# 0xMiden/miden-vm

Hardware: AMD Instinct MI355X
Metric: trace rows/sec proved (2^20-row trace, 96-bit sec) (higher is better)
Workload: dtype u64 (Goldilocks field, p = 2^64 - 2^32 + 1); 1 GPU; full proof of miden:20:51:8 (DummyMidenAir 2^20 x 51 + 8 EF aux), 96-bit production PCS params (blowup 8, FRI arity 4, 27 queries, PoW 4/12/16), Poseidon2 LMCS; trace resident in HBM, transcript on host; log_trace_rows=20, main_width=51, aux_width_ef=8, log_blowup=3, proof_bytes=137697, parallelism=1 GPU

## Files before the change

miden-vm_amd/csrc/ntt.hip:

```cpp
#include "ctx.hpp"
#include "gl.cuh"
#include "kernels.hpp"
#include "poseidon2_fast.cuh"
#include <utility>

#ifndef NTT_ASM_MUL
#define NTT_ASM_MUL 2
#endif
#if P2F_ASM && NTT_ASM_MUL == 1
#define NTT_MUL1 p2f_mul
#elif P2F_ASM && NTT_ASM_MUL == 2
#define NTT_MUL1 p2f_mul_nv
#else
#define NTT_MUL1 p2f_mul_c
#endif

static constexpr int NTT_TILE_LOG = 12;
static constexpr int NTT_TILE_LOG_BIG = 14;
static constexpr int NTT_THREADS = 256;
static int ntt_tile_log(int log_n) {
  static const int big_max = [] {
    const char* e = getenv("MH_NTT_BIG_MAX");
    return e ? atoi(e) : 22;
  }();
  return log_n > 20 && log_n <= big_max ? NTT_TILE_LOG_BIG : NTT_TILE_LOG;
}

static bool ntt_coef_rot(int log_n) {
  static const int on = [] { const char* e = getenv("MH_NTT_ROT"); return e ? atoi(e) : 1; }();
  return on && log_n >= NTT_TILE_LOG && ntt_tile_log(log_n) == NTT_TILE_LOG;
}

struct PowTable {
  u64 pw[32];
};
__global__ void k_fill_powers(u64* out, size_t n, PowTable t, u64 scale) {
  size_t k = blockIdx.x * (size_t)blockDim.x + threadIdx.x;
  if (k >= n) return;
  u64 r = scale;
  size_t e = k;
#pragma unroll 1
  for (int i = 0; e; i++, e >>= 1)
    if (e & 1) r = gl_mul(r, t.pw[i]);
  out[k] = r;
}

static void fill_powers(mh_ctx* c, u64* out, size_t n, u64 base, u64 scale) {
  PowTable t;
  u64 b = base;
  for (int i = 0; i < 32; i++) {
    t.pw[i] = b;
    b = gl_sqr(b);
  }
  if (n == 0) return;
  MH_LAUNCH(k_fill_powers, dim3((n + 255) / 256), dim3(256), 0, c->stream, out, n, t, scale);
}

const u64* mh_ctx::twiddles(int log_n, bool inverse) {
  auto& m = inverse ? tw_inv : tw_fwd;
  auto it = m.find(log_n);
  if (it != m.end()) return it->second.u();
  size_t half = log_n ? ((size_t)1 << (log_n - 1)) : 1;
  DevBuf b(half * 8);
  u64 w = gl_two_adic_generator(log_n);
  if (inverse) w = gl_inv(w);
  fill_powers(this, b.u(), half, w, 1);
  const u64* p = b.u();
  m[log_n] = std::move(b);
  return p;
}

__global__ __launch_bounds__(256) void k_transpose_rm_to_cm(const u64* __restrict__ in, u64* __restrict__ out, size_t n,
                                                           size_t w) {
  __shared__ u64 tile[32][33];
  size_t r0 = (size_t)blockIdx.x * 32, c0 = (size_t)blockIdx.y * 32;
  int tx = threadIdx.x & 31, ty = threadIdx.x >> 5;
  for (int k = ty; k < 32; k += 8) {
    size_t r = r0 + k, cc = c0 + tx;
    if (r < n && cc < w) tile[k][tx] = in[r * w + cc];
  }
  __syncthreads();
  for (int k = ty; k < 32; k += 8) {
    size_t cc = c0 + k, r = r0 + tx;
    if (r < n && cc < w) out[cc * n + r] = gl_canon(tile[tx][k]);
  }
}

void launch_transpose_rm_to_cm(mh_ctx* c, const u64* in, u64* out, size_t n, size_t w, hipStream_t stream) {
  dim3 grid((unsigned)((n + 31) / 32), (unsigned)((w + 31) / 32));
  MH_LAUNCH(k_transpose_rm_to_cm, grid, dim3(256), 0, stream ? stream : c->stream, in, out, n, w);
}

struct NttPassArgs {
  const u64* src;
// ... 344 lines not shown
    t[i] = NttW{v0[f], v1[f], v2[f]};
    if (!INV) {
      if (S) t[i] = ntt_w_shl(pre ? ntt_w_from(ntt_w_fold1(ntt_w_bias(t[i]))) : t[i], S);
      p[i] = a[i];
      q[i] = t[i];
    } else {
      p[i] = E >= 96 ? t[i] : a[i];
      q[i] = E >= 96 ? a[i] : t[i];
    }
  }
  ntt_w_bflyN<N>(s, d, a, t, p, q);
#pragma unroll
  for (int i = 0; i < N; i++) {
    const int e = ntt_bfly_lo(M, K0 + i), f = e | (1 << M), j = e & ((1 << M) - 1);
    const int E = (W16 * (8 >> M) * j) % 192, S = E % 96;
    const bool pre = (FOLD >> (8 * M + j)) & 1u;
    NttW lo = s[i], hi = d[i];
    if (!INV) {
      if (E >= 96) { lo = d[i]; hi = s[i]; }
    } else if (S) {
      hi = ntt_w_shl(pre ? ntt_w_from(ntt_w_fold1(ntt_w_bias(hi))) : hi, S);
    }
    v0[e] = lo.w0; v1[e] = lo.w1; v2[e] = lo.w2;
    v0[f] = hi.w0; v1[f] = hi.w1; v2[f] = hi.w2;
  }
}
template <int G, bool INV, int I = 0>
__device__ __forceinline__ void ntt_w_stages(u32 (&v0)[1 << G], u32 (&v1)[1 << G], u32 (&v2)[1 << G]) {
  if constexpr (I < G) {
    constexpr int M = INV ? G - 1 - I : I, H = 1 << (G - 1), N = H < NTT_ILV ? H : NTT_ILV;
    ntt_w_stage_part<G, INV, M, 0, N>(v0, v1, v2);
    if constexpr (H > N) ntt_w_stage_part<G, INV, M, N, H - N>(v0, v1, v2);
    ntt_w_stages<G, INV, I + 1>(v0, v1, v2);
  }
}
template <int G, bool INV>
__device__ __forceinline__ void ntt_dft_wide(u64 (&x)[1 << G]) {
  u32 v0[1 << G], v1[1 << G], v2[1 << G];
#pragma unroll
  for (int e = 0; e < (1 << G); e++) { v0[e] = lo32(x[e]); v1[e] = hi32(x[e]); v2[e] = 0u; }
  const NttW z = ntt_w_bias(NttW{v0[0], v1[0], 0u});
  v0[0] = z.w0; v1[0] = z.w1; v2[0] = z.w2;
  ntt_w_stages<G, INV>(v0, v1, v2);
  constexpr int NF = (1 << G) < NTT_ILV ? (1 << G) : NTT_ILV;
#pragma unroll
  for (int c = 0; c < (1 << G); c += NF) {
    u64 r[NF];
    u32 f0[NF], f1[NF], f2[NF];
#pragma unroll
    for (int i = 0; i < NF; i++) { f0[i] = v0[c + i]; f1[i] = v1[c + i]; f2[i] = v2[c + i]; }
    ntt_w_foldN<NF>(r, f0, f1, f2);
#pragma unroll
    for (int i = 0; i < NF; i++) x[c + i] = r[i];
  }
}
#endif

template <int G, bool INV>
__device__ __forceinline__ void ntt_dft_regs(u64 (&x)[1 << G], bool dif) {
#if P2F_ASM && NTT_ASM_BFLY == 2
  ntt_dft_wide<G, INV>(x);
  return;
#elif P2F_ASM && NTT_ASM_BFLY
  if constexpr (!INV && G >= 3) {
    ntt_fwd_dft_asm<G>(x);
    return;
  }
#endif
  constexpr int W16 = INV ? 36 : 156;
  if (!dif) {
#pragma unroll
    for (int m = 0; m < G; m++)
#pragma unroll
      for (int e = 0; e < (1 << G); e++)
        if (!(e & (1 << m))) ntt_bfly_dit(x[e], x[e | (1 << m)], (W16 * (8 >> m) * (e & ((1 << m) - 1))) % 192);
  } else {
#pragma unroll
    for (int m = G - 1; m >= 0; m--)
#pragma unroll
      for (int e = 0; e < (1 << G); e++)
        if (!(e & (1 << m))) ntt_bfly_dif(x[e], x[e | (1 << m)], (W16 * (8 >> m) * (e & ((1 << m) - 1))) % 192);
  }
}
template <int K, int OFF>
__device__ __forceinline__ void ntt_tw_mul(u64* x, const u64* __restrict__ tw, int s, u32 gm) {
  if constexpr (K > 0) {
    constexpr int C = K >= 5 ? 5 : K;
    u64 a[C], b[C];
#pragma unroll
    for (int i = 0; i < C; i++) {
      a[i] = x[OFF + i];
      b[i] = (tw + ((size_t)(OFF + i - 1) << s))[gm];
    }
#if P2F_ASM && NTT_ASM_MUL == 1
    p2f_mulN<C>(a, a, b);
#else
#pragma unroll
    for (int i = 0; i < C; i++) a[i] = NTT_MUL1(a[i], b[i]);
#endif
#pragma unroll
    for (int i = 0; i < C; i++) x[OFF + i] = a[i];
    ntt_tw_mul<K - C, OFF + C>(x, tw, s, gm);
  }
}
#else
template <int K, int OFF>
__device__ void ntt_tw_mul(u64* x, const u64* __restrict__ tw, int s, u32 gm);
template <int G, bool INV>
__device__ void ntt_dft_regs(u64 (&x)[1 << G], bool dif);
__device__ u64 ntt_canon(u64 t);
__device__ u64 p2f_mul_c(u64 a, u64 b);
#endif

#ifndef NTT16_OCC
#define NTT16_OCC
#endif
#ifndef NTT_SWZ
#define NTT_SWZ 1
#endif
static size_t ntt_lds_bytes(int tile_log) {
  if (NTT_SWZ && tile_log == NTT_TILE_LOG) return ((size_t)1 << tile_log) * 8;
  return (((size_t)1 << tile_log) + ((size_t)1 << (tile_log - 4))) * 8;
}
template <bool SWZ>
__device__ __forceinline__ u32 ntt_pad(u32 l) {
  return SWZ ? (l ^ ((l >> 4) & 31u)) : (l + (l >> 4));
}

#define NTT_STORE(p, v) (*(p) = (v))
template <int G, bool INV, bool SWZ, int B0>
__device__ __forceinline__ void ntt_round(const NttPassArgs& a, u64* lds, int st, u32 tile_n, size_t lo0, u64* dst_direct,
                                          size_t gbase, const u64* __restrict__ tw, const u64* __restrict__ src_direct = nullptr,
                                          const u64* xin = nullptr) {
  const int b0 = B0 >= 0 ? B0 : st + a.cb, s = a.s_lo + st;
  const u32 cb_mask = (1u << a.cb) - 1;
  constexpr bool FAST = SWZ && B0 >= 0;
  for (u32 q = threadIdx.x; q < (tile_n >> G); q += blockDim.x) {
    const u32 low = q & ((1u << b0) - 1);
    const u32 l0 = ((q >> b0) << (b0 + G)) | low;
    const u32 gm = (((l0 >> a.cb) & ((1u << st) - 1)) << a.s_lo) | ((u32)lo0 << a.cb) | (l0 & cb_mask);
    const u32 p0 = ntt_pad<SWZ>(l0);
    char* const ldsb = reinterpret_cast<char*>(lds);
    const u32 pb = p0 * 8u, pb1 = (p0 ^ 16u) * 8u;
    auto slot = [&](int e) -> u64* {
      if constexpr (FAST && B0 == 8) return reinterpret_cast<u64*>(ldsb + ((e & 1) ? pb1 : pb) + ((u32)e << 11));
      else if constexpr (FAST) return reinterpret_cast<u64*>(ldsb + (pb ^ (ntt_pad<true>((u32)e << B0) * 8u)));
      else return lds + (SWZ ? (p0 ^ ntt_pad<true>((u32)e << b0)) : ntt_pad<false>(l0 | ((u32)e << b0)));
    };
    u64 x[1 << G];
    if (xin) {
#pragma unroll
      for (int e = 0; e < (1 << G); e++) x[e] = xin[e];
    } else if (src_direct) {
      const u32 six = (u32)(gbase | ((size_t)(l0 >> a.cb) << a.s_lo) | (l0 & cb_mask));
#pragma unroll
      for (int e = 0; e < (1 << G); e++) x[e] = (src_direct + ((size_t)e << s))[six];
    } else {
#pragma unroll
    for (int e = 0; e < (1 << G); e++) x[e] = *slot(e);
    }
    if (!INV && s > 0) ntt_tw_mul<(1 << G) - 1, 1>(x, tw, s, gm);
    ntt_dft_regs<G, INV>(x, INV);
    if (INV && s > 0) ntt_tw_mul<(1 << G) - 1, 1>(x, tw, s, gm);
    if (INV && dst_direct && a.rot && b0 == 0 && G == 4) {
      const u32 rix = (u32)gbase + (l0 >> 4);
#pragma unroll
      for (int e = 0; e < (1 << G); e++) NTT_STORE((dst_direct + ((size_t)e << 8)) + rix, a.canon_out ? ntt_canon(x[e]) : x[e]);
    } else if (dst_direct) {
      const u32 tix = (u32)(gbase | ((size_t)(l0 >> a.cb) << a.s_lo) | (l0 & cb_mask));
      if (a.canon_out) {
#pragma unroll
        for (int e = 0; e < (1 << G); e++) NTT_STORE((dst_direct + ((size_t)e << s)) + tix, ntt_canon(x[e]));
      } else {
#pragma unroll
        for (int e = 0; e < (1 << G); e++) NTT_STORE((dst_direct + ((size_t)e << s)) + tix, x[e]);
      }
    } else {
#pragma unroll
      for (int e = 0; e < (1 << G); e++) *slot(e) = x[e];
    }
  }
}

template <bool INV, int THREADS, int MODE = 0>
__global__ __launch_bounds__(THREADS) NTT16_OCC void k_ntt16_pass(NttPassArgs a) {
  extern __shared__ u64 lds[];
  constexpr bool SWZ = NTT_SWZ && THREADS == NTT_THREADS;
  const int tile_log = a.r_bits + a.cb;
  const u32 tile_n = 1u << tile_log;
  const u32 cb_mask = (1u << a.cb) - 1;
  const u32 tile = a.col_fastest ? blockIdx.y : blockIdx.x;
  const u32 col_id = a.col_fastest ? blockIdx.x : blockIdx.y;
  const int lo_bits = a.s_lo - a.cb;
  const size_t lo0 = tile & ((1u << lo_bits) - 1);
  const size_t hi = tile >> lo_bits;
  const size_t gbase = (hi << (a.s_lo + a.r_bits)) | (lo0 << a.cb);
  const u64* src0 = a.src + (size_t)col_id * a.src_col_stride;
  u64 raw[MODE == 1 ? 16 : 1];
  for (u32 z = 0; z < a.n_z; z++) {
  const u32 zc = blockIdx.z * a.n_z + z;
  const u32 srow = a.group_cols ? (col_id / a.group_cols) * a.group_z + zc : zc;
  u64* dst = a.dst + (size_t)col_id * a.dst_col_stride + (size_t)zc * a.dst_z_stride;
  const u64* src = src0 + (size_t)zc * a.src_z_stride;
  if (z) __syncthreads();

  constexpr int LOG_T = THREADS == 256 ? 8 : 10;
  const bool direct_first = MODE == 0 && THREADS == NTT_THREADS && a.direct_first && tile_n == 16u * THREADS;
  if (direct_first) {
  } else if (tile_n == 16u * THREADS && a.cb <= LOG_T) {
    const u32 tid = threadIdx.x;
    const u32 g0 = (u32)(gbase | ((size_t)(tid >> a.cb) << a.s_lo) | (tid & cb_mask));
    const int shg = LOG_T - a.cb + a.s_lo;
    const u32 p0 = ntt_pad<SWZ>(tid);
    if constexpr (MODE == 1) {
      if (z == 0) {
#pragma unroll
        for (int j = 0; j < 16; j++) raw[j] = (src + ((size_t)j << shg))[g0];
        if (a.scale_full) {
          const u64* sf = a.scale_full + ((size_t)srow << a.log_n);
#pragma unroll
          for (int c = 0; c < 16; c += 4) {
            u64 t[4];
#pragma unroll
            for (int j = 0; j < 4; j++) t[j] = (sf + ((size_t)(c + j) << shg))[g0];
#pragma unroll
            for (int j = 0; j < 4; j++) raw[c + j] = NTT_MUL1(raw[c + j], t[j]);
          }
        } else {
#pragma unroll 4
          for (int j = 0; j < 16; j++) {
            const u32 k = bitrev32(a.rot ? (g0 - tid) + ((tid << 4) | (u32)j) : g0 + ((u32)j << shg), a.log_n);
            const u64 sc = NTT_MUL1(a.scale_lo[srow * a.scale_lo_z + (k & ((1u << a.lb) - 1))], a.scale_hi[srow * a.scale_hi_z + (k >> a.lb)]);
            raw[j] = NTT_MUL1(raw[j], sc);
          }
        }
      } else {
#pragma unroll
        for (int c = 0; c < 16; c += 8) {
          u64 t[8];
#pragma unroll
          for (int j = 0; j < 8; j++) t[j] = (a.step + ((size_t)(c + j) << shg))[g0];
#pragma unroll
          for (int j = 0; j < 8; j++) raw[c + j] = NTT_MUL1(raw[c + j], t[j]);
        }
      }
      if (!a.rot) {
#pragma unroll
        for (int j = 0; j < 16; j++) lds[p0 ^ ntt_pad<true>((u32)j * THREADS)] = raw[j];
      }
    } else
    if (THREADS == NTT_THREADS && !a.scale_lo && !a.scale_full) {
      u64 v[16];
#pragma unroll
      for (int j = 0; j < 16; j++) v[j] = (src + ((size_t)j << shg))[g0];
#pragma unroll
      for (int j = 0; j < 16; j++)
        lds[SWZ ? (p0 ^ ntt_pad<true>((u32)j * THREADS)) : ntt_pad<false>(tid + (u32)j * THREADS)] = v[j];
    } else
#pragma unroll 1
    for (int c = 0; c < 16; c += 4) {
      u64 v[4];
#pragma unroll
      for (int j = 0; j < 4; j++) v[j] = (src + ((size_t)(c + j) << shg))[g0];
      if (a.scale_full) {
        const u64* sf = a.scale_full + ((size_t)srow << a.log_n);
#pragma unroll
        for (int j = 0; j < 4; j++) v[j] = NTT_MUL1(v[j], (sf + ((size_t)(c + j) << shg))[g0]);
      } else if (a.scale_lo) {
#pragma unroll
        for (int j = 0; j < 4; j++) {
          const u32 k = bitrev32(a.rot ? (g0 - tid) + ((tid << 4) | (u32)(c + j)) : g0 + ((u32)(c + j) << shg), a.log_n);
          const u64 sc = NTT_MUL1(a.scale_lo[srow * a.scale_lo_z + (k & ((1u << a.lb) - 1))], a.scale_hi[srow * a.scale_hi_z + (k >> a.lb)]);
          v[j] = NTT_MUL1(v[j], sc);
        }
      }
      if (a.rot) {
#pragma unroll
        for (int j = 0; j < 4; j++) lds[ntt_pad<SWZ>((tid << 4) | (u32)(c + j))] = v[j];
      } else
#pragma unroll
      for (int j = 0; j < 4; j++)
        lds[SWZ ? (p0 ^ ntt_pad<true>((u32)(c + j) * THREADS)) : ntt_pad<false>(tid + (u32)(c + j) * THREADS)] = v[j];
    }
  } else {
    for (u32 l = threadIdx.x; l < tile_n; l += THREADS) {
      size_t g = gbase | ((size_t)(l >> a.cb) << a.s_lo) | (l & cb_mask);
      u64 v = src[g];
      if (a.scale_full) {
        v = NTT_MUL1(v, a.scale_full[((size_t)srow << a.log_n) + g]);
      } else if (a.scale_lo) {
        u32 k = bitrev32((u32)g, a.log_n);
        u64 sc = NTT_MUL1(a.scale_lo[srow * a.scale_lo_z + (k & ((1u << a.lb) - 1))], a.scale_hi[srow * a.scale_hi_z + (k >> a.lb)]);
        v = NTT_MUL1(v, sc);
      }
      lds[ntt_pad<SWZ>(l)] = v;
    }
  }
  const bool regs_first = MODE == 1 && a.rot;
  if (!direct_first && !regs_first) __syncthreads();
  const int rem = a.r_bits & 3, n16 = a.r_bits >> 2;
  const int n_rounds = n16 + (rem ? 1 : 0);
  if (n_rounds == 0) {
    if (threadIdx.x == 0) dst[gbase] = ntt_canon(lds[0]);
    continue;
  }
  for (int i = 0; i < n_rounds; i++) {
    const int ri = INV ? n_rounds - 1 - i : i;
    int st, g;
    if (rem) {
      st = ri == 0 ? 0 : rem + 4 * (ri - 1);
      g = ri == 0 ? rem : 4;
    } else {
      st = 4 * ri;
      g = 4;
    }
    u64* direct = (i == n_rounds - 1) ? dst : nullptr;
    const int b0 = st + a.cb;
#define NTT_ROUND(GG, BB) ntt_round<GG, INV, SWZ, BB>(a, lds, st, tile_n, lo0, direct, gbase, a.tw_round[ri])
    if (direct_first && i == 0) ntt_round<4, INV, SWZ, INV ? 8 : 4>(a, lds, st, tile_n, lo0, direct, gbase, a.tw_round[ri], src);
    else if (regs_first && i == 0) ntt_round<4, INV, SWZ, 0>(a, lds, st, tile_n, lo0, direct, gbase, a.tw_round[ri], nullptr, raw);
    else if (g == 4 && b0 == 0) NTT_ROUND(4, 0);
    else if (g == 4 && b0 == 4) NTT_ROUND(4, 4);
    else if (g == 4 && b0 == 8) NTT_ROUND(4, 8);
    else if (g == 4) NTT_ROUND(4, -1);
    else if (g == 3) NTT_ROUND(3, -1);
    else if (g == 2) NTT_ROUND(2, -1);
    else NTT_ROUND(1, -1);
#undef NTT_ROUND
    if (!direct) __syncthreads();
  }
  }
}

struct PassPlan {
  int s_lo, r_bits, cb;
};
static std::vector<PassPlan> plan_passes(int log_n) {
  std::vector<PassPlan> p;
  const int T = ntt_tile_log(log_n);
  int c = log_n < T ? log_n : T;
  p.push_back({0, c, 0});
  int rem = log_n - c;
  if (rem > 0) {
    const int max_r = T - 4;
    int np = (rem + max_r - 1) / max_r;
    int s = c;
    for (int i = 0; i < np; i++) {
      int r = rem / np + (i < rem % np ? 1 : 0);
      p.push_back({s, r, T - r});
      s += r;
    }
  }
  return p;
}

static std::vector<std::pair<int, int>> pass_rounds(int r_bits) {
  std::vector<std::pair<int, int>> r;
  const int rem = r_bits & 3;
  int st = 0;
  if (rem) {
    r.push_back({0, rem});
    st = rem;
  }
  for (; st < r_bits; st += 4) r.push_back({st, 4});
  return r;
}
__global__ void k_fill_round_plane(u64* out, int s, int G, int log_n, PowTable t) {
  const size_t idx = blockIdx.x * (size_t)blockDim.x + threadIdx.x;
  if (idx >= ((size_t)((1 << G) - 1) << s)) return;
  const u32 e = (u32)(idx >> s) + 1;
  const size_t gm = idx & (((size_t)1 << s) - 1);
  const u32 rho = bitrev32(e, G);
  size_t ex = (gm * rho) << (log_n - s - G);
  u64 r = 1;
#pragma unroll 1
  for (int i = 0; ex; i++, ex >>= 1)
    if (ex & 1) r = gl_mul(r, t.pw[i]);
  out[idx] = r;
}
struct NttPlanes {
  const u64* base;
  std::vector<size_t> off;
};
static NttPlanes ntt_planes(mh_ctx* c, int log_n, bool inverse, const std::vector<PassPlan>& plan) {
  const std::string key = "nttp:" + std::to_string(log_n) + (inverse ? ":i" : ":f");
  auto it = c->tables.find(key);
  if (it == c->tables.end()) {
    std::vector<size_t> off(plan.size() * 4, 0);
    size_t total = 1;
    for (size_t i = 0; i < plan.size(); i++) {
      auto rounds = pass_rounds(plan[i].r_bits);
      for (size_t k = 0; k < rounds.size(); k++) {
        const int s = plan[i].s_lo + rounds[k].first, G = rounds[k].second;
        off[i * 4 + k] = total;
        if (s > 0) total += (size_t)((1 << G) - 1) << s;
      }
    }
    DevBuf b(total * 8);
    PowTable t;
    u64 w = gl_two_adic_generator(log_n);
    if (inverse) w = gl_inv(w);
    for (int i = 0; i < 32; i++) {
      t.pw[i] = w;
      w = gl_sqr(w);
    }
    for (size_t i = 0; i < plan.size(); i++) {
      auto rounds = pass_rounds(plan[i].r_bits);
      for (size_t k = 0; k < rounds.size(); k++) {
        const int s = plan[i].s_lo + rounds[k].first, G = rounds[k].second;
        if (s == 0) continue;
        const size_t cnt = (size_t)((1 << G) - 1) << s;
        MH_LAUNCH(k_fill_round_plane, dim3((unsigned)((cnt + 255) / 256)), dim3(256), 0, c->stream, b.u() + off[i * 4 + k], s, G,
                           log_n, t);
      }
    }
    c->table_index[key] = off;
    it = c->tables.emplace(key, std::move(b)).first;
  }
  return NttPlanes{it->second.u(), c->table_index[key]};
}

static void launch_pass(mh_ctx* c, NttPassArgs a, size_t n_cols, size_t n_z, bool one_coset_per_workgroup = false) {
  size_t tiles = (size_t)1 << (a.log_n - a.r_bits - a.cb);
  MH_REQUIRE(n_z >= 1 && (n_z & (n_z - 1)) == 0, "internal: the number of output cosets of a pass must be a power of two");
  size_t zsplit = 1;
  while (zsplit < n_z && (one_coset_per_workgroup || tiles * n_cols * zsplit < 4096)) zsplit *= 2;
  a.n_z = (u32)(n_z / zsplit);
  static const int colfast = [] { const char* e = getenv("MH_NTT_COLFAST"); return e ? atoi(e) : 1; }();
  a.col_fastest = (colfast && tiles <= 65535) ? 1 : 0;
  dim3 grid(a.col_fastest ? (unsigned)n_cols : (unsigned)tiles, a.col_fastest ? (unsigned)tiles : (unsigned)n_cols, (unsigned)zsplit);
  const int T = ntt_tile_log(a.log_n);
  const size_t lds = ntt_lds_bytes(T);
  if (T == NTT_TILE_LOG) {
    if (a.dif) MH_LAUNCH((k_ntt16_pass<true, NTT_THREADS>), grid, dim3(NTT_THREADS), lds, c->stream, a);
    else if (a.step && a.n_z > 1 && NTT_SWZ && a.r_bits + a.cb == NTT_TILE_LOG && a.cb == 0)
      MH_LAUNCH((k_ntt16_pass<false, NTT_THREADS, 1>), grid, dim3(NTT_THREADS), lds, c->stream, a);
    else MH_LAUNCH((k_ntt16_pass<false, NTT_THREADS>), grid, dim3(NTT_THREADS), lds, c->stream, a);
  } else {
    if (!c->ntt_big_lds_attr) {
      HIP_CHECK(hipFuncSetAttribute((const void*)k_ntt16_pass<true, 1024>, hipFuncAttributeMaxDynamicSharedMemorySize, (int)lds));
      HIP_CHECK(hipFuncSetAttribute((const void*)k_ntt16_pass<false, 1024>, hipFuncAttributeMaxDynamicSharedMemorySize, (int)lds));
      c->ntt_big_lds_attr = true;
    }
    if (a.dif) MH_LAUNCH((k_ntt16_pass<true, 1024>), grid, dim3(1024), lds, c->stream, a);
    else MH_LAUNCH((k_ntt16_pass<false, 1024>), grid, dim3(1024), lds, c->stream, a);
  }
}

void ntt_inverse_dif_inplace(mh_ctx* c, u64* cols, size_t n_cols, int log_n) { ntt_inverse_dif(c, cols, cols, n_cols, log_n); }

void ntt_inverse_dif(mh_ctx* c, const u64* src, u64* dst, size_t n_cols, int log_n) {
  if (log_n == 0) {
    if (src != dst) HIP_CHECK(hipMemcpyAsync(dst, src, n_cols * 8, hipMemcpyDeviceToDevice, c->stream));
    return;
  }
  auto plan = plan_passes(log_n);
  const NttPlanes tw = ntt_planes(c, log_n, true, plan);
  for (int i = (int)plan.size() - 1; i >= 0; i--) {
    NttPassArgs a{};
    a.src = (i == (int)plan.size() - 1) ? src : dst; a.dst = dst;
    a.src_col_stride = a.dst_col_stride = (size_t)1 << log_n;
    a.dst_z_stride = 0;
    a.log_n = log_n; a.s_lo = plan[i].s_lo; a.r_bits = plan[i].r_bits; a.cb = plan[i].cb;
    a.dif = 1; a.scale_lo = nullptr; a.scale_hi = nullptr;
    for (int k = 0; k < 4; k++) a.tw_round[k] = tw.base + tw.off[i * 4 + k];
    a.canon_out = 0;
    static const int direct = [] { const char* e = getenv("MH_NTT_DIRECT"); return e ? atoi(e) : 1; }();
    a.direct_first = direct && NTT_SWZ && a.r_bits >= 4 && a.r_bits + a.cb == NTT_TILE_LOG;
    a.rot = i == 0 && ntt_coef_rot(log_n);
    launch_pass(c, a, n_cols, 1);
  }
}

struct CosetTables {
  const u64* lo;
  const u64* hi;
  int lb;
};
static CosetTables coset_tables(mh_ctx* c, int log_n, const std::vector<u64>& bases, u64 post_scale) {
  CosetTables t;
  t.lb = (log_n + 1) / 2;
  const size_t nlo = (size_t)1 << t.lb, nhi = (size_t)1 << (log_n - t.lb);
  u64 h = 0xcbf29ce484222325ULL ^ (u64)log_n;
  for (u64 b : bases) h = (h ^ b) * 0x100000001b3ULL + (h >> 29);
  h = (h ^ post_scale) * 0x100000001b3ULL;
  const std::string key = "coset:" + std::to_string(log_n) + ":" + std::to_string(bases.size()) + ":" + std::to_string(h);
  auto it = c->tables.find(key);
  if (it == c->tables.end()) {
    DevBuf b((bases.size() * (nlo + nhi)) * 8);
    for (size_t z = 0; z < bases.size(); z++) {
      fill_powers(c, b.u() + z * nlo, nlo, bases[z], 1);
      fill_powers(c, b.u() + bases.size() * nlo + z * nhi, nhi, gl_exp_pow2(bases[z], t.lb), post_scale);
    }
    std::vector<size_t> ident(bases.begin(), bases.end());
    ident.push_back((size_t)post_scale);
    c->table_index[key] = ident;
    it = c->tables.emplace(key, std::move(b)).first;
  } else {
    const std::vector<size_t>& ident = c->table_index[key];
    bool same = ident.size() == bases.size() + 1 && ident.back() == (size_t)post_scale;
    for (size_t z = 0; same && z < bases.size(); z++) same = ident[z] == (size_t)bases[z];
    MH_REQUIRE(same, "internal: coset table key collision");
  }
  t.lo = it->second.u();
  t.hi = it->second.u() + bases.size() * nlo;
  return t;
}

__global__ void k_fill_scale_full(u64* out, const u64* lo, const u64* hi, int log_n, int lb, size_t lo_z, size_t hi_z, int rot) {
  const size_t i = blockIdx.x * (size_t)blockDim.x + threadIdx.x;
  const size_t n = (size_t)1 << log_n;
  const size_t z = blockIdx.y;
  if (i >= n) return;
  const u32 il = rot ? (((u32)i & ~4095u) | (((u32)i & 255u) << 4) | (((u32)i >> 8) & 15u)) : (u32)i;
  const u32 k = bitrev32(il, log_n);
  out[z * n + i] = gl_mul(lo[z * lo_z + (k & ((1u << lb) - 1))], hi[z * hi_z + (k >> lb)]);
}
static const u64* coset_scale_full(mh_ctx* c, int log_n, const std::vector<u64>& bases, u64 post_scale, const CosetTables& t) {
  const int rot = ntt_coef_rot(log_n) ? 1 : 0;
// ... 123 lines not shown
```

miden-vm_amd/csrc/poseidon2_fast.cuh:

```cuda
#pragma once
#include "poseidon2.cuh"

namespace p2c {
#include "p2_fast_constants.inc"
}

#ifndef P2F_ASM
#define P2F_ASM 1
#endif
#ifndef P2F_GROUP
#define P2F_GROUP 4
#endif
#ifndef P2F_RC_ADDEND
#define P2F_RC_ADDEND 1
#endif
#if !P2F_ASM
#undef P2F_RC_ADDEND
#define P2F_RC_ADDEND 0
#endif
#ifndef P2F_TAILS
#define P2F_TAILS 1
#endif

#if defined(__HIP_DEVICE_COMPILE__)
// ... 72 lines not shown
    if constexpr (BS) P2F_MAD0S(i, m[i], lo32(a[i]), hi32(b[i]));
    else if constexpr (KA) P2F_MADK(i, m[i], lo32(a[i]), hi32(b[i]), ka[2 * i + 1]);
    else P2F_MAD0(i, m[i], lo32(a[i]), hi32(b[i]));
  }
#pragma unroll
  for (int i = 0; i < N; i++) {
    if constexpr (BS) P2F_A("v_mad_u64_u32 %0, %1, %2, %3, %4" : "=v"(m[i]), "=s"(cm[i]) : "v"(hi32(a[i])), "s"(lo32(b[i])), "0"(m[i]));
    else P2F_A("v_mad_u64_u32 %0, %1, %2, %3, %4" : "=v"(m[i]), "=s"(cm[i]) : "v"(hi32(a[i])), "v"(lo32(b[i])), "0"(m[i]));
  }
#pragma unroll
  for (int i = 0; i < N; i++) P2F_A("v_add_co_u32_e64 %0, %1, %2, %3" : "=v"(w1[i]), "=s"(k1[i]) : "v"(hi32(p00[i])), "v"(lo32(m[i])));
  P2F_GAP();
#pragma unroll
  for (int i = 0; i < N; i++) P2F_A("v_addc_co_u32_e64 %0, %1, %2, 0, %3" : "=v"(accl[i]), "=s"(k2[i]) : "v"(hi32(m[i])), "s"(k1[i]));
#pragma unroll
  for (int i = 0; i < N; i++)
    k3[i] = cm[i] | k2[i];
#pragma unroll
  for (int i = 0; i < N; i++) {
    const u32 zero = 0;
    P2F_CARRY_IN(i, "v_addc_co_u32_e64", acch[i], zero, k3[i]);
  }
#pragma unroll
  for (int i = 0; i < N; i++) {
    const u64 acc = ((u64)acch[i] << 32) | accl[i];
    if constexpr (BS) P2F_MADAS(i, hi[i], hi32(a[i]), hi32(b[i]), acc);
    else P2F_MADA(i, hi[i], hi32(a[i]), hi32(b[i]), acc);
  }
#pragma unroll
  for (int i = 0; i < N; i++) {
    const u64 lo = ((u64)w1[i] << 32) | lo32(p00[i]);
    P2F_A("v_mad_u64_u32 %0, %1, %2, -1, %3" : "=v"(t[i]), "=s"(c1[i]) : "v"(lo32(hi[i])), "v"(lo));
  }
  P2F_GAP();
#pragma unroll
  for (int i = 0; i < N; i++) P2F_A("v_subb_co_u32_e64 %0, %1, %2, %3, %4" : "=v"(rl[i]), "=s"(bb[i]) : "v"(lo32(t[i])), "v"(hi32(hi[i])), "s"(c1[i]));
#pragma unroll
  for (int i = 0; i < N; i++) P2F_CARRY_IN(i, "v_addc_co_u32_e64", rh[i], hi32(t[i]), c1[i]);
  if (P2F_GAP_NOPS && N == 1) P2F_A("s_nop 0");
#pragma unroll
  for (int i = 0; i < N; i++) P2F_A("v_subb_co_u32_e64 %0, %1, %2, 0, %3" : "=v"(rh[i]), "=s"(bw[i]) : "0"(rh[i]), "s"(bb[i]));
  P2F_GAP();
#pragma unroll
  for (int i = 0; i < N; i++) P2F_A("v_addc_co_u32_e64 %0, %1, %2, 0, %3" : "=v"(rl[i]), "=s"(c3[i]) : "0"(rl[i]), "s"(bw[i]));
#pragma unroll
  for (int i = 0; i < N; i++) k3[i] = bw[i] & ~c3[i];
#pragma unroll
  for (int i = 0; i < N; i++) {
    P2F_CARRY_IN(i, "v_subb_co_u32_e64", rh[i], rh[i], k3[i]);
    r[i] = ((u64)rh[i] << 32) | rl[i];
  }
}
#undef P2F_GAP
#undef P2F_SCR
#undef P2F_MAD0
#undef P2F_MADA
#undef P2F_MAD0S
#undef P2F_MADAS
#undef P2F_MADK
#undef P2F_CARRY_IN
__device__ __forceinline__ u64 p2f_mul_nv(u64 a, u64 b) {
  u64 p00, m, hi, t, d0, d1, d2, d3, d4, d5, cm, k1, k2, c1, bb, bw, c3;
  u32 w1, accl, acch, rl, rh;
  const u32 zero = 0;
  asm("v_mad_u64_u32 %0, %1, %2, %3, 0" : "=v"(p00), "=s"(d0) : "v"(lo32(a)), "v"(lo32(b)));
  asm("v_mad_u64_u32 %0, %1, %2, %3, 0" : "=v"(m), "=s"(d1) : "v"(lo32(a)), "v"(hi32(b)));
  asm("v_mad_u64_u32 %0, %1, %2, %3, %4" : "=v"(m), "=s"(cm) : "v"(hi32(a)), "v"(lo32(b)), "0"(m));
  asm("v_add_co_u32_e64 %0, %1, %2, %3" : "=v"(w1), "=s"(k1) : "v"(hi32(p00)), "v"(lo32(m)));
  asm("s_nop 1\n\tv_addc_co_u32_e64 %0, %1, %2, 0, %3" : "=v"(accl), "=s"(k2) : "v"(hi32(m)), "s"(k1));
  const u64 k3 = cm | k2;
  asm("v_addc_co_u32_e64 %0, %1, %2, 0, %3" : "=v"(acch), "=s"(d2) : "v"(zero), "s"(k3));
  const u64 acc = ((u64)acch << 32) | accl;
  asm("v_mad_u64_u32 %0, %1, %2, %3, %4" : "=v"(hi), "=s"(d3) : "v"(hi32(a)), "v"(hi32(b)), "v"(acc));
  const u64 lo = ((u64)w1 << 32) | lo32(p00);
  asm("v_mad_u64_u32 %0, %1, %2, -1, %3" : "=v"(t), "=s"(c1) : "v"(lo32(hi)), "v"(lo));
  asm("s_nop 1\n\tv_subb_co_u32_e64 %0, %1, %2, %3, %4" : "=v"(rl), "=s"(bb) : "v"(lo32(t)), "v"(hi32(hi)), "s"(c1));
  asm("s_nop 1\n\tv_addc_co_u32_e64 %0, %1, %2, 0, %3" : "=v"(rh), "=s"(d4) : "v"(hi32(t)), "s"(c1));
  asm("s_nop 1\n\tv_subb_co_u32_e64 %0, %1, %2, 0, %3" : "=v"(rh), "=s"(bw) : "0"(rh), "s"(bb));
  asm("s_nop 1\n\tv_addc_co_u32_e64 %0, %1, %2, 0, %3" : "=v"(rl), "=s"(c3) : "0"(rl), "s"(bw));
  const u64 mk = bw & ~c3;
  asm("v_subb_co_u32_e64 %0, %1, %2, 0, %3" : "=v"(rh), "=s"(d5) : "0"(rh), "s"(mk));
  return ((u64)rh << 32) | rl;
}
__device__ __forceinline__ u64 p2f_mul(u64 a, u64 b) {
#if P2F_ASM
  u64 r[1];
  const u64 x[1] = {a}, y[1] = {b};
  p2f_mulN<1>(r, x, y);
  return r[0];
#else
  return p2f_mul_c(a, b);
#endif
}
__device__ __forceinline__ u64 p2f_mul_k(u64 a, u64 k) {
#if P2F_ASM
  u64 r[1];
  const u64 x[1] = {a}, y[1] = {k};
  p2f_mulN<1, true>(r, x, y);
  return r[0];
#else
  return p2f_mul_c(a, k);
#endif
}
__device__ __forceinline__ u64 p2f_sbox(u64 x) {
#if P2F_ASM
  const u64 x2 = p2f_mul(x, x);
  u64 q[2];
  const u64 qa[2] = {x2, x2}, qb[2] = {x, x2};
  p2f_mulN<2>(q, qa, qb);
  return p2f_mul(q[0], q[1]);
#else
  const u64 x2 = p2f_mul(x, x);
  const u64 x3 = p2f_mul(x2, x);
  const u64 x4 = p2f_mul(x2, x2);
  return p2f_mul(x3, x4);
#endif
}
template <int W>
__device__ __forceinline__ void p2f_load_k(unsigned long long (&d)[W], const unsigned long long* k) {
  if constexpr (W == 8) {
    typedef unsigned long long k8 __attribute__((ext_vector_type(8)));
    const k8 v = *reinterpret_cast<const k8*>(k);
#pragma unroll
    for (int i = 0; i < 8; i++) d[i] = v[i];
  } else {
#pragma unroll
    for (int i = 0; i < W; i++) d[i] = k[i];
  }
}
template <bool KA = false>
__device__ __forceinline__ void p2f_sbox12(u64 s[12], const unsigned long long* k = nullptr) {
#if P2F_ASM
#pragma unroll
  for (int g = 0; g < 12; g += P2F_GROUP) {
    u64 x[P2F_GROUP], x2[P2F_GROUP], x3[P2F_GROUP];
#pragma unroll
    for (int i = 0; i < P2F_GROUP; i++) x[i] = s[g + i];
    p2f_mulN<P2F_GROUP>(x2, x, x);
    p2f_mulN<P2F_GROUP>(x3, x2, x);
    p2f_mulN<P2F_GROUP>(x, x2, x2);
    if constexpr (KA) {
      unsigned long long kg[2 * P2F_GROUP];
      p2f_load_k(kg, k + 2 * g);
      p2f_mulN<P2F_GROUP, false, true>(x2, x3, x, kg);
    } else {
      p2f_mulN<P2F_GROUP>(x2, x3, x);
    }
#pragma unroll
    for (int i = 0; i < P2F_GROUP; i++) s[g + i] = x2[i];
  }
#else
  static_assert(!KA, "addends need the asm form of the product");
#pragma unroll
  for (int i = 0; i < 12; i++) s[i] = p2f_sbox(s[i]);
#endif
}
__device__ __forceinline__ u64 p2f_add_canon(u64 x, u64 c) {
  u64 s = x + c;
  s += (s < c) ? GL_EPS : 0;
  return s;
}
__device__ __forceinline__ u64 p2f_fold(u64 L, u64 H) {
  const u64 m = (u64)hi32(H) * 0xFFFFFFFFu + L;
  const u32 hl = lo32(H);
  const u32 s = hi32(m) + hl;
  u64 r = ((u64)s << 32) | lo32(m);
// ... 297 lines not shown
```

Before: 25.00 million trace rows/s.

## Interleave grouped Goldilocks multiplies in asm and specialise two forward NTT pass shapes

Measured after the change: 25.26 million trace rows/s (median of 6 runs). +1.0%, better.

```diff
diff --git a/miden-vm_amd/csrc/ntt.hip b/miden-vm_amd/csrc/ntt.hip
--- a/miden-vm_amd/csrc/ntt.hip
+++ b/miden-vm_amd/csrc/ntt.hip
@@ -5,11 +5,14 @@
 #include <utility>
 
 #ifndef NTT_ASM_MUL
-#define NTT_ASM_MUL 2
+#define NTT_ASM_MUL 3
+#endif
+#ifndef NTT_MUL_GROUP
+#define NTT_MUL_GROUP 3
 #endif
 #if P2F_ASM && NTT_ASM_MUL == 1
 #define NTT_MUL1 p2f_mul
-#elif P2F_ASM && NTT_ASM_MUL == 2
+#elif P2F_ASM && NTT_ASM_MUL >= 2
 #define NTT_MUL1 p2f_mul_nv
 #else
 #define NTT_MUL1 p2f_mul_c
@@ -520,30 +523,45 @@
         if (!(e & (1 << m))) ntt_bfly_dif(x[e], x[e | (1 << m)], (W16 * (8 >> m) * (e & ((1 << m) - 1))) % 192);
   }
 }
-template <int K, int OFF>
+template <int C, bool GRP, bool TW = false>
+__device__ __forceinline__ void ntt_mulN(u64 (&a)[C], const u64 (&b)[C]) {
+#if P2F_ASM && NTT_ASM_MUL == 3
+  if constexpr (GRP && C >= 3 && C <= 5) {
+    p2f_mulN_nv<C>(a, a, b);
+    return;
+  }
+#elif P2F_ASM && NTT_ASM_MUL == 1
+  if constexpr (TW) {
+    p2f_mulN<C>(a, a, b);
+    return;
+  }
+#endif
+#pragma unroll
+  for (int i = 0; i < C; i++) a[i] = NTT_MUL1(a[i], b[i]);
+}
+template <int K, int OFF, bool GRP>
 __device__ __forceinline__ void ntt_tw_mul(u64* x, const u64* __restrict__ tw, int s, u32 gm) {
   if constexpr (K > 0) {
-    constexpr int C = K >= 5 ? 5 : K;
+    constexpr bool F3 = NTT_ASM_MUL == 3 && GRP;
+    constexpr int M = F3 ? NTT_MUL_GROUP : 5, R = K - M;
+    constexpr int C = K <= M ? K : (F3 && (R == 1 || R == 2) && K - 3 >= 3 && K - 3 <= 5) ? K - 3 : M;
     u64 a[C], b[C];
 #pragma unroll
     for (int i = 0; i < C; i++) {
       a[i] = x[OFF + i];
       b[i] = (tw + ((size_t)(OFF + i - 1) << s))[gm];
     }
-#if P2F_ASM && NTT_ASM_MUL == 1
-    p2f_mulN<C>(a, a, b);
+    ntt_mulN<C, GRP, true>(a, b);
+#pragma unroll
+    for (int i = 0; i < C; i++) x[OFF + i] = a[i];
+    ntt_tw_mul<K - C, OFF + C, GRP>(x, tw, s, gm);
+  }
+}
 #else
-#pragma unroll
-    for (int i = 0; i < C; i++) a[i] = NTT_MUL1(a[i], b[i]);
-#endif
-#pragma unroll
-    for (int i = 0; i < C; i++) x[OFF + i] = a[i];
-    ntt_tw_mul<K - C, OFF + C>(x, tw, s, gm);
-  }
-}
-#else
-template <int K, int OFF>
+template <int K, int OFF, bool GRP>
 __device__ void ntt_tw_mul(u64* x, const u64* __restrict__ tw, int s, u32 gm);
+template <int C, bool GRP, bool TW = false>
+__device__ void ntt_mulN(u64 (&a)[C], const u64 (&b)[C]);
 template <int G, bool INV>
 __device__ void ntt_dft_regs(u64 (&x)[1 << G], bool dif);
 __device__ u64 ntt_canon(u64 t);
@@ -566,7 +584,7 @@
 }
 
 #define NTT_STORE(p, v) (*(p) = (v))
-template <int G, bool INV, bool SWZ, int B0>
+template <int G, bool INV, bool SWZ, int B0, bool GRP = !INV>
 __device__ __forceinline__ void ntt_round(const NttPassArgs& a, u64* lds, int st, u32 tile_n, size_t lo0, u64* dst_direct,
                                           size_t gbase, const u64* __restrict__ tw, const u64* __restrict__ src_direct = nullptr,
                                           const u64* xin = nullptr) {
@@ -597,9 +615,9 @@
 #pragma unroll
     for (int e = 0; e < (1 << G); e++) x[e] = *slot(e);
     }
-    if (!INV && s > 0) ntt_tw_mul<(1 << G) - 1, 1>(x, tw, s, gm);
+    if (!INV && s > 0) ntt_tw_mul<(1 << G) - 1, 1, GRP>(x, tw, s, gm);
     ntt_dft_regs<G, INV>(x, INV);
-    if (INV && s > 0) ntt_tw_mul<(1 << G) - 1, 1>(x, tw, s, gm);
+    if (INV && s > 0) ntt_tw_mul<(1 << G) - 1, 1, GRP>(x, tw, s, gm);
     if (INV && dst_direct && a.rot && b0 == 0 && G == 4) {
       const u32 rix = (u32)gbase + (l0 >> 4);
 #pragma unroll
@@ -620,10 +638,28 @@
   }
 }
 
-template <bool INV, int THREADS, int MODE = 0>
-__global__ __launch_bounds__(THREADS) NTT16_OCC void k_ntt16_pass(NttPassArgs a) {
+template <int SHAPE>
+__device__ __forceinline__ void ntt_shape_consts(NttPassArgs& a) {
+  if constexpr (SHAPE != 0) {
+    a.dif = 0; a.step = nullptr;
+  }
+  if constexpr (SHAPE == 1) {
+    a.s_lo = 0; a.r_bits = NTT_TILE_LOG; a.cb = 0; a.rot = 1; a.direct_first = 0;
+    a.src_z_stride = 0;
+  } else if constexpr (SHAPE == 2) {
+    a.r_bits = 8; a.cb = 4; a.rot = 0; a.direct_first = 1; a.canon_out = 1;
+    a.scale_lo = a.scale_hi = a.scale_full = nullptr;
+    a.group_cols = a.group_z = 0; a.lb = 0; a.scale_lo_z = a.scale_hi_z = 0;
+  }
+}
+template <bool INV, int THREADS, int MODE = 0, int SHAPE = 0>
+__global__ __launch_bounds__(THREADS) NTT16_OCC void k_ntt16_pass(NttPassArgs a_in) {
+  static_assert(SHAPE == 0 || (!INV && THREADS == NTT_THREADS && MODE == 0 && NTT_SWZ), "the two specialised bodies are forward passes on the 2^12 tile");
+  NttPassArgs a = a_in;
+  ntt_shape_consts<SHAPE>(a);
   extern __shared__ u64 lds[];
   constexpr bool SWZ = NTT_SWZ && THREADS == NTT_THREADS;
+  constexpr bool GRP = !INV && MODE == 0;
   const int tile_log = a.r_bits + a.cb;
   const u32 tile_n = 1u << tile_log;
   const u32 cb_mask = (1u << a.cb) - 1;
@@ -687,7 +723,7 @@
         for (int j = 0; j < 16; j++) lds[p0 ^ ntt_pad<true>((u32)j * THREADS)] = raw[j];
       }
     } else
-    if (THREADS == NTT_THREADS && !a.scale_lo && !a.scale_full) {
+    if (SHAPE != 1 && THREADS == NTT_THREADS && !a.scale_lo && !a.scale_full) {
       u64 v[16];
 #pragma unroll
       for (int j = 0; j < 16; j++) v[j] = (src + ((size_t)j << shg))[g0];
@@ -702,15 +738,20 @@
       for (int j = 0; j < 4; j++) v[j] = (src + ((size_t)(c + j) << shg))[g0];
       if (a.scale_full) {
         const u64* sf = a.scale_full + ((size_t)srow << a.log_n);
-#pragma unroll
-        for (int j = 0; j < 4; j++) v[j] = NTT_MUL1(v[j], (sf + ((size_t)(c + j) << shg))[g0]);
+        u64 t[4];
+#pragma unroll
+        for (int j = 0; j < 4; j++) t[j] = (sf + ((size_t)(c + j) << shg))[g0];
+        ntt_mulN<4, GRP>(v, t);
       } else if (a.scale_lo) {
+        u64 sl[4], sh[4];
 #pragma unroll
         for (int j = 0; j < 4; j++) {
           const u32 k = bitrev32(a.rot ? (g0 - tid) + ((tid << 4) | (u32)(c + j)) : g0 + ((u32)(c + j) << shg), a.log_n);
-          const u64 sc = NTT_MUL1(a.scale_lo[srow * a.scale_lo_z + (k & ((1u << a.lb) - 1))], a.scale_hi[srow * a.scale_hi_z + (k >> a.lb)]);
-          v[j] = NTT_MUL1(v[j], sc);
+          sl[j] = a.scale_lo[srow * a.scale_lo_z + (k & ((1u << a.lb) - 1))];
+          sh[j] = a.scale_hi[srow * a.scale_hi_z + (k >> a.lb)];
         }
+        ntt_mulN<4, GRP>(sl, sh);
+        ntt_mulN<4, GRP>(v, sl);
       }
       if (a.rot) {
 #pragma unroll
@@ -742,7 +783,7 @@
     if (threadIdx.x == 0) dst[gbase] = ntt_canon(lds[0]);
     continue;
   }
-  for (int i = 0; i < n_rounds; i++) {
+  auto round = [&](int i) __attribute__((always_inline)) {
     const int ri = INV ? n_rounds - 1 - i : i;
     int st, g;
     if (rem) {
@@ -754,9 +795,9 @@
     }
     u64* direct = (i == n_rounds - 1) ? dst : nullptr;
     const int b0 = st + a.cb;
-#define NTT_ROUND(GG, BB) ntt_round<GG, INV, SWZ, BB>(a, lds, st, tile_n, lo0, direct, gbase, a.tw_round[ri])
-    if (direct_first && i == 0) ntt_round<4, INV, SWZ, INV ? 8 : 4>(a, lds, st, tile_n, lo0, direct, gbase, a.tw_round[ri], src);
-    else if (regs_first && i == 0) ntt_round<4, INV, SWZ, 0>(a, lds, st, tile_n, lo0, direct, gbase, a.tw_round[ri], nullptr, raw);
+#define NTT_ROUND(GG, BB) ntt_round<GG, INV, SWZ, BB, GRP>(a, lds, st, tile_n, lo0, direct, gbase, a.tw_round[ri])
+    if (direct_first && i == 0) ntt_round<4, INV, SWZ, INV ? 8 : 4, GRP>(a, lds, st, tile_n, lo0, direct, gbase, a.tw_round[ri], src);
+    else if (regs_first && i == 0) ntt_round<4, INV, SWZ, 0, GRP>(a, lds, st, tile_n, lo0, direct, gbase, a.tw_round[ri], nullptr, raw);
     else if (g == 4 && b0 == 0) NTT_ROUND(4, 0);
     else if (g == 4 && b0 == 4) NTT_ROUND(4, 4);
     else if (g == 4 && b0 == 8) NTT_ROUND(4, 8);
@@ -766,6 +807,13 @@
     else NTT_ROUND(1, -1);
 #undef NTT_ROUND
     if (!direct) __syncthreads();
+  };
+  if constexpr (SHAPE == 1) {
+    round(0); round(1); round(2);
+  } else if constexpr (SHAPE == 2) {
+    round(0); round(1);
+  } else {
+    for (int i = 0; i < n_rounds; i++) round(i);
   }
   }
 }
@@ -873,6 +921,10 @@
     if (a.dif) MH_LAUNCH((k_ntt16_pass<true, NTT_THREADS>), grid, dim3(NTT_THREADS), lds, c->stream, a);
     else if (a.step && a.n_z > 1 && NTT_SWZ && a.r_bits + a.cb == NTT_TILE_LOG && a.cb == 0)
       MH_LAUNCH((k_ntt16_pass<false, NTT_THREADS, 1>), grid, dim3(NTT_THREADS), lds, c->stream, a);
+    else if (NTT_SWZ && a.s_lo == 0 && a.r_bits == NTT_TILE_LOG && a.cb == 0 && a.rot && a.scale_lo && !a.step && !a.direct_first && !a.src_z_stride)
+      MH_LAUNCH((k_ntt16_pass<false, NTT_THREADS, 0, 1>), grid, dim3(NTT_THREADS), lds, c->stream, a);
+    else if (NTT_SWZ && a.direct_first && a.r_bits == 8 && a.cb == 4 && a.canon_out && !a.rot && !a.scale_lo && !a.scale_full && !a.step && !a.group_cols)
+      MH_LAUNCH((k_ntt16_pass<false, NTT_THREADS, 0, 2>), grid, dim3(NTT_THREADS), lds, c->stream, a);
     else MH_LAUNCH((k_ntt16_pass<false, NTT_THREADS>), grid, dim3(NTT_THREADS), lds, c->stream, a);
   } else {
     if (!c->ntt_big_lds_attr) {
diff --git a/miden-vm_amd/csrc/poseidon2_fast.cuh b/miden-vm_amd/csrc/poseidon2_fast.cuh
--- a/miden-vm_amd/csrc/poseidon2_fast.cuh
+++ b/miden-vm_amd/csrc/poseidon2_fast.cuh
@@ -178,6 +178,128 @@
   asm("v_subb_co_u32_e64 %0, %1, %2, 0, %3" : "=v"(rh), "=s"(d5) : "0"(rh), "s"(mk));
   return ((u64)rh << 32) | rl;
 }
+#define P2F_NV_STAGE_(TXT, OUT, IN, DD)                                                                                            \
+  do {                                                                                                                             \
+    if constexpr (C == 3) asm(TXT(0) TXT(1) TXT(2) : OUT(0), OUT(1), OUT(2) DD : IN(0), IN(1), IN(2));                             \
+    else if constexpr (C == 4) asm(TXT(0) TXT(1) TXT(2) TXT(3) : OUT(0), OUT(1), OUT(2), OUT(3) DD : IN(0), IN(1), IN(2), IN(3));  \
+    else asm(TXT(0) TXT(1) TXT(2) TXT(3) TXT(4) : OUT(0), OUT(1), OUT(2), OUT(3), OUT(4) DD : IN(0), IN(1), IN(2), IN(3), IN(4));  \
+  } while (0)
+#define P2F_NV_NODD
+#define P2F_NV_DD , [dd] "=&s"(dd)
+#define P2F_NV_STAGE(TXT, OUT, IN) P2F_NV_STAGE_(TXT, OUT, IN, P2F_NV_NODD)
+#define P2F_NV_STAGE_D(TXT, OUT, IN) P2F_NV_STAGE_(TXT, OUT, IN, P2F_NV_DD)
+template <int C>
+__device__ __forceinline__ void p2f_mulN_nv(u64 (&r)[C], const u64 (&a)[C], const u64 (&b)[C]) {
+  static_assert(C >= 3 && C <= 5, "fewer than 3 products do not cover the wait states; more than 5 exceed an asm statement's operands");
+  u64 p00[C], m[C], hi[C], t[C], acc[C], lo[C], dd;
+  u64 cm[C], k1[C], k2[C], k3[C], c1[C], bb[C], bw[C], c3[C];
+  u32 w1[C], accl[C], acch[C], rl[C], rh[C];
+#define NV_T(i) "v_mad_u64_u32 %[d" #i "], %[dd], %[x" #i "], %[y" #i "], 0\n\t"
+#define NV_O(i) [d##i] "=&v"(p00[i])
+#define NV_I(i) [x##i] "v"(lo32(a[i])), [y##i] "v"(lo32(b[i]))
+  P2F_NV_STAGE_D(NV_T, NV_O, NV_I);
+#undef NV_O
+#undef NV_I
+#define NV_O(i) [d##i] "=&v"(m[i])
+#define NV_I(i) [x##i] "v"(lo32(a[i])), [y##i] "v"(hi32(b[i]))
+  P2F_NV_STAGE_D(NV_T, NV_O, NV_I);
+#undef NV_T
+#undef NV_O
+#undef NV_I
+#define NV_T(i) "v_mad_u64_u32 %[d" #i "], %[c" #i "], %[x" #i "], %[y" #i "], %[d" #i "]\n\t"
+#define NV_O(i) [d##i] "+&v"(m[i]), [c##i] "=&s"(cm[i])
+#define NV_I(i) [x##i] "v"(hi32(a[i])), [y##i] "v"(lo32(b[i]))
+  P2F_NV_STAGE(NV_T, NV_O, NV_I);
+#undef NV_T
+#undef NV_O
+#undef NV_I
+#define NV_T(i) "v_add_co_u32_e64 %[d" #i "], %[c" #i "], %[x" #i "], %[y" #i "]\n\t"
+#define NV_O(i) [d##i] "=&v"(w1[i]), [c##i] "=&s"(k1[i])
+#define NV_I(i) [x##i] "v"(hi32(p00[i])), [y##i] "v"(lo32(m[i]))
+  P2F_NV_STAGE(NV_T, NV_O, NV_I);
+#undef NV_T
+#undef NV_O
+#undef NV_I
+#define NV_T(i) "v_addc_co_u32_e64 %[d" #i "], %[c" #i "], %[x" #i "], 0, %[k" #i "]\n\t"
+#define NV_O(i) [d##i] "=&v"(accl[i]), [c##i] "=&s"(k2[i])
+#define NV_I(i) [x##i] "v"(hi32(m[i])), [k##i] "s"(k1[i])
+  P2F_NV_STAGE(NV_T, NV_O, NV_I);
+#undef NV_T
+#undef NV_O
+#undef NV_I
+#pragma unroll
+  for (int i = 0; i < C; i++) k3[i] = cm[i] | k2[i];
+#define NV_T(i) "v_addc_co_u32_e64 %[d" #i "], %[dd], 0, 0, %[k" #i "]\n\t"
+#define NV_O(i) [d##i] "=&v"(acch[i])
+#define NV_I(i) [k##i] "s"(k3[i])
+  P2F_NV_STAGE_D(NV_T, NV_O, NV_I);
+#undef NV_T
+#undef NV_O
+#undef NV_I
+#pragma unroll
+  for (int i = 0; i < C; i++) {
+    acc[i] = ((u64)acch[i] << 32) | accl[i];
+    lo[i] = ((u64)w1[i] << 32) | lo32(p00[i]);
+  }
+#define NV_T(i) "v_mad_u64_u32 %[d" #i "], %[dd], %[x" #i "], %[y" #i "], %[z" #i "]\n\t"
+#define NV_O(i) [d##i] "=&v"(hi[i])
+#define NV_I(i) [x##i] "v"(hi32(a[i])), [y##i] "v"(hi32(b[i])), [z##i] "v"(acc[i])
+  P2F_NV_STAGE_D(NV_T, NV_O, NV_I);
+#undef NV_T
+#undef NV_O
+#undef NV_I
+#define NV_T(i) "v_mad_u64_u32 %[d" #i "], %[c" #i "], %[x" #i "], -1, %[z" #i "]\n\t"
+#define NV_O(i) [d##i] "=&v"(t[i]), [c##i] "=&s"(c1[i])
+#define NV_I(i) [x##i] "v"(lo32(hi[i])), [z##i] "v"(lo[i])
+  P2F_NV_STAGE(NV_T, NV_O, NV_I);
+#undef NV_T
+#undef NV_O
+#undef NV_I
+#define NV_T(i) "v_subb_co_u32_e64 %[d" #i "], %[c" #i "], %[x" #i "], %[y" #i "], %[k" #i "]\n\t"
+#define NV_O(i) [d##i] "=&v"(rl[i]), [c##i] "=&s"(bb[i])
+#define NV_I(i) [x##i] "v"(lo32(t[i])), [y##i] "v"(hi32(hi[i])), [k##i] "s"(c1[i])
+  P2F_NV_STAGE(NV_T, NV_O, NV_I);
+#undef NV_T
+#undef NV_O
+#undef NV_I
+#define NV_T(i) "v_addc_co_u32_e64 %[d" #i "], %[dd], %[x" #i "], 0, %[k" #i "]\n\t"
+#define NV_O(i) [d##i] "=&v"(rh[i])
+#define NV_I(i) [x##i] "v"(hi32(t[i])), [k##i] "s"(c1[i])
+  P2F_NV_STAGE_D(NV_T, NV_O, NV_I);
+#undef NV_T
+#undef NV_O
+#undef NV_I
+#define NV_T(i) "v_subb_co_u32_e64 %[d" #i "], %[c" #i "], %[d" #i "], 0, %[k" #i "]\n\t"
+#define NV_O(i) [d##i] "+&v"(rh[i]), [c##i] "=&s"(bw[i])
+#define NV_I(i) [k##i] "s"(bb[i])
+  P2F_NV_STAGE(NV_T, NV_O, NV_I);
+#undef NV_T
+#undef NV_O
+#define NV_T(i) "v_addc_co_u32_e64 %[d" #i "], %[c" #i "], %[d" #i "], 0, %[k" #i "]\n\t"
+#define NV_O(i) [d##i] "+&v"(rl[i]), [c##i] "=&s"(c3[i])
+#undef NV_I
+#define NV_I(i) [k##i] "s"(bw[i])
+  P2F_NV_STAGE(NV_T, NV_O, NV_I);
+#undef NV_T
+#undef NV_O
+#undef NV_I
+#pragma unroll
+  for (int i = 0; i < C; i++) k3[i] = bw[i] & ~c3[i];
+#define NV_T(i) "v_subb_co_u32_e64 %[d" #i "], %[dd], %[d" #i "], 0, %[k" #i "]\n\t"
+#define NV_O(i) [d##i] "+&v"(rh[i])
+#define NV_I(i) [k##i] "s"(k3[i])
+  P2F_NV_STAGE_D(NV_T, NV_O, NV_I);
+#undef NV_T
+#undef NV_O
+#undef NV_I
+#pragma unroll
+  for (int i = 0; i < C; i++) r[i] = ((u64)rh[i] << 32) | rl[i];
+}
+#undef P2F_NV_STAGE_
+#undef P2F_NV_STAGE
+#undef P2F_NV_STAGE_D
+#undef P2F_NV_NODD
+#undef P2F_NV_DD
 __device__ __forceinline__ u64 p2f_mul(u64 a, u64 b) {
 #if P2F_ASM
   u64 r[1];
```
